# aanna0701/face-recognition-pytorch

Measured on AMD Instinct MI355X. Metric: train imgs/sec IR-50-layout ResNet50 + ArcFace/PartialFC head, 112x112, higher is better.
Workload: dtype bf16

## Files before the change

face-recognition-pytorch_amd/frhip/csrc/igemm_halo.hip:

```cpp
#include "igemm_halo.h"
#include "igemm_halo_wide.h"
#include "frhip.h"

namespace frhip {

#ifndef FRHIP_CLOCK_STAMP
#define FRHIP_CLOCK_STAMP 0
#endif
#if FRHIP_CLOCK_STAMP
__device__ unsigned long long g_clock_stamps[2 * 8192];
#endif

template <typename T, int WM, int WN, int MT, int HBUFS, bool XF = false, bool LEAN = false>
__device__ __forceinline__ void halo_body(const HaloGeom& g, const void* __restrict__ a, const void* __restrict__ b,
                                          void* __restrict__ out, const void* __restrict__ res, float* __restrict__ stats,
                                          const EpiBnRed& br, char* smem, int mtile, int ntile) {
    typedef HaloTile<T, WM, WN, MT, HBUFS> Tile;
    HaloMainloop<T, WM, WN, MT, HBUFS, XF> ml;
#if FRHIP_CLOCK_STAMP
    const unsigned long long t0 = __builtin_amdgcn_s_memtime(), r0 = __builtin_amdgcn_s_memrealtime();
#endif
    ml.run(g, a, b, smem, mtile, ntile);
#if FRHIP_CLOCK_STAMP
    if (threadIdx.x == 0) {
        const unsigned long long t1 = __builtin_amdgcn_s_memtime(), r1 = __builtin_amdgcn_s_memrealtime();
        g_clock_stamps[2 * (blockIdx.x & 8191)] = t1 - t0;
        g_clock_stamps[2 * (blockIdx.x & 8191) + 1] = r1 - r0;
    }
#endif
    if constexpr (FRHIP_ABL & 16) {
        if (g.M >= 0) {
#pragma unroll
            for (int i = 0; i < 4; ++i)
#pragma unroll
                for (int j = 0; j < MT; ++j) asm volatile("" :: "v"(ml.acc[i][j]));
            return;
        }
    }
    const int wave = wave_id();
    const int wm = wave / WN, wn = wave % WN;
    const int m0 = mtile * Tile::BM + wm * Tile::WROWS, n0 = ntile * Tile::BN + wn * 64;
    EpiOperands<T, Tile::WROWS> eo;
    if constexpr (LEAN) {
        eo.fetch_fast(res, stats ? br.y : nullptr, g.M, g.Nout, m0, n0);
        const char* mine = ml.template stage_out<T>(smem);
        nt_epilogue_store_fast<T, WM, WN, Tile::WROWS, Tile::THREADS, Tile::BN>(mine, Tile::template stage_pitch<T>(), smem, g.M, g.Nout,
                                                                                out, res != nullptr, stats, br, eo, mtile, ntile);
    } else {
        eo.fetch(res, (stats || br.gelu_bwd) ? br.y : nullptr, g.M, g.Nout, m0, n0, br.res_h, br.res_w, &br.map);
        const char* mine = ml.template stage_out<T>(smem);
        nt_epilogue_store<T, WM, WN, Tile::WROWS, Tile::THREADS, Tile::BN>(mine, Tile::template stage_pitch<T>(), smem, g.M, g.Nout,
                                                                           out, res != nullptr, stats, br, eo, mtile, ntile, m0, n0);
    }
}

template <typename T, int WM, int WN, int MT, int HBUFS, bool XF = false, bool LEAN = false>
__global__ __launch_bounds__(64 * WM * WN, 2) void halo_kernel(HaloGeom g, const void* __restrict__ a,
                                                                         const void* __restrict__ b, void* __restrict__ out,
                                                                         const void* __restrict__ res, float* __restrict__ stats,
                                                                         EpiBnRed br, int mtiles, int ntiles) {
    extern __shared__ __attribute__((aligned(16))) char smem[];
    const uint32_t lin = xcd_remap(blockIdx.x, gridDim.x);
    const int ntile = (int)(lin % (uint32_t)ntiles), mtile = (int)(lin / (uint32_t)ntiles);
    halo_body<T, WM, WN, MT, HBUFS, XF, LEAN>(g, a, b, out, res, stats, br, smem, mtile, ntile);
}

template <bool LEAN>
__global__ __launch_bounds__(256, 2) void halo_wide_kernel(HaloGeom g, const void* __restrict__ a, const void* __restrict__ b,
                                                           void* __restrict__ out, const void* __restrict__ res,
                                                           float* __restrict__ stats, EpiBnRed br, int mtiles, int ntiles) {
    typedef HaloWideTile Tile;
    typedef bf16_t T;
    extern __shared__ __attribute__((aligned(16))) char smem[];
    const uint32_t lin = xcd_remap(blockIdx.x, gridDim.x);
    const int ntile = (int)(lin % (uint32_t)ntiles), mtile = (int)(lin / (uint32_t)ntiles);
    const int m_tile0 = mtile * Tile::BM;
    HaloWideMainloop ml;
#if FRHIP_CLOCK_STAMP
    const unsigned long long t0 = __builtin_amdgcn_s_memtime(), r0 = __builtin_amdgcn_s_memrealtime();
#endif
    ml.run(g, a, b, smem, m_tile0, ntile);
#if FRHIP_CLOCK_STAMP
    if (threadIdx.x == 0) {
        const unsigned long long t1 = __builtin_amdgcn_s_memtime(), r1 = __builtin_amdgcn_s_memrealtime();
        g_clock_stamps[2 * (blockIdx.x & 8191)] = t1 - t0;
        g_clock_stamps[2 * (blockIdx.x & 8191) + 1] = r1 - r0;
    }
#endif
    const int m0 = m_tile0 + wave_id() * Tile::WROWS;
#pragma unroll
    for (int half = 0; half < 2; ++half) {
        const int n0 = ntile * Tile::BN + half * 64;
        EpiOperands<T, Tile::WROWS> eo;
        if constexpr (LEAN) {
            eo.fetch_fast(res, stats ? br.y : nullptr, g.M, g.Nout, m0, n0);
            const char* mine = ml.stage_out(smem, half);
            nt_epilogue_store_fast<T, 4, 1, Tile::WROWS, Tile::THREADS, 64>(mine, Tile::stage_pitch, smem, g.M, g.Nout, out, res != nullptr,
                                                                            stats, br, eo, mtile, ntile * 2 + half);
        } else {
            eo.fetch(res, (stats || br.gelu_bwd) ? br.y : nullptr, g.M, g.Nout, m0, n0, br.res_h, br.res_w, &br.map);
            const char* mine = ml.stage_out(smem, half);
            nt_epilogue_store<T, 4, 1, Tile::WROWS, Tile::THREADS, 64>(mine, Tile::stage_pitch, smem, g.M, g.Nout, out, res != nullptr,
                                                                       stats, br, eo, mtile, ntile * 2 + half, m0, n0);
        }
    }
}

int g_epi_lean = 1;

bool halo_lean_pick(int family, long long M, int Nout, const EpiBnRed& br) {
    if (family == HALO_WIDE) return g_epi_lean && epi_lean_ok(true, M, Nout, HaloWideTile::BM, HaloWideTile::BN, br);
    typedef HaloTile<bf16_t, 4, 1, 4, 1> Tile;
    return family == HALO_4WAVE && g_epi_lean && epi_lean_ok(true, M, Nout, Tile::BM, Tile::BN, br);
}

static int halo_wide_launch(const HaloGeom& g, const void* a, const void* b, void* out, const void* res, float* stats,
                            const EpiBnRed& br, hipStream_t stream) {
    typedef HaloWideTile Tile;
    const int mtiles = (g.M + Tile::BM - 1) / Tile::BM, ntiles = (g.Nout + Tile::BN - 1) / Tile::BN;
    const bool lean = halo_lean_pick(HALO_WIDE, g.M, g.Nout, br);
    auto kern = lean ? halo_wide_kernel<true> : halo_wide_kernel<false>;
    if (set_dynamic_lds(reinterpret_cast<const void*>(kern), Tile::LDS, "igemm_halo")) return FRHIP_ELAUNCH;
    hipLaunchKernelGGL(kern, dim3(mtiles * ntiles), dim3(Tile::THREADS), Tile::LDS, stream, g, a, b, out, res, stats, br, mtiles, ntiles);
    return check_launch("igemm_halo_wide");
}

template <typename T, int WM, int WN, int MT, int HBUFS, bool XF = false>
static int halo_launch(const HaloGeom& g, const void* a, const void* b, void* out, const void* res, float* stats,
                       const EpiBnRed& br, hipStream_t stream) {
    typedef HaloTile<T, WM, WN, MT, HBUFS> Tile;
    const int mtiles = (g.M + Tile::BM - 1) / Tile::BM, ntiles = (g.Nout + Tile::BN - 1) / Tile::BN;
    const int lds = Tile::template lds_bytes<T>();
    constexpr bool HAS_LEAN = sizeof(T) == 2 && WM == 4 && WN == 1 && MT == 4 && HBUFS == 1;
    bool lean = false;
    if constexpr (HAS_LEAN) lean = halo_lean_pick(HALO_4WAVE, g.M, g.Nout, br);
    auto kern = halo_kernel<T, WM, WN, MT, HBUFS, XF, false>;
    if constexpr (HAS_LEAN) { if (lean) kern = halo_kernel<T, WM, WN, MT, HBUFS, XF, true>; }
    if (set_dynamic_lds(reinterpret_cast<const void*>(kern), lds, "igemm_halo")) return FRHIP_ELAUNCH;
    hipLaunchKernelGGL(kern, dim3(mtiles * ntiles), dim3(Tile::THREADS), lds, stream, g, a, b, out, res, stats, br, mtiles, ntiles);
    return check_launch("igemm_halo");
}

static int g_halo_enabled = 1;

bool halo_applicable(int dtype, int h, int w, int c, int k, int r, int s, int stride, int pad) {
    const int bke = NT_ROWB / (dtype == FRHIP_DT_BF16 ? 2 : 4);
    return g_halo_enabled && r == 3 && s == 3 && stride == 1 && pad == 1 && w <= 56 && (c % bke) == 0 && (k % 8) == 0 &&
           (dtype == FRHIP_DT_BF16 || dtype == FRHIP_DT_F32);
}

static int g_halo_wide_dirs = 2;
static int halo_config(int dtype, int c, int k);
static int halo_config_w(int dtype, int w, int c, int k, int sign) {
    if ((g_halo_wide_dirs & (sign > 0 ? 1 : 2)) && dtype == FRHIP_DT_BF16 && w <= HaloWideTile::MAXW &&
        (k % 128) == 0 && (c % 64) == 0 && c >= 128 && (g_halo_enabled & 3) == 1)
        return 3;
    return halo_config(dtype, c, k);
}
static int halo_config(int dtype, int c, int k) {
    const int es = dtype == FRHIP_DT_BF16 ? 2 : 4;
    const int nchunks = c / (NT_ROWB / es);
    const bool narrow = (k % 128) != 0;
    if (dtype == FRHIP_DT_BF16) {
        const int mode = g_halo_enabled & 3;
        const bool two_per_cu = mode == 2 || (mode != 3 && nchunks <= 8);
        if (two_per_cu || narrow) return (nchunks == 1 || two_per_cu) ? 0 : 1;
        return 2;
    }
    return narrow ? 1 : 2;
}

int halo_family(int dtype, int w, int c, int k, int sign) {
    if (halo_config_w(dtype, w, c, k, sign) == 3) return HALO_WIDE;
    const int cfg = halo_config(dtype, c, k);
    if (dtype == FRHIP_DT_BF16 && cfg == 0) return HALO_4WAVE;
    return cfg == 1 ? HALO_8X1 : HALO_4X2;
}

bool halo_lean_applies(int dtype, int n, int h, int w, int c, int k, int sign) {
    if (!g_epi_lean || dtype != FRHIP_DT_BF16) return false;
    const long long M = 1LL * n * h * w;
    const int cfg = halo_config_w(dtype, w, c, k, sign) == 3 ? 3 : halo_config(dtype, c, k);
    const int bn = cfg == 3 ? HaloWideTile::BN : 64;
    if (cfg != 3 && cfg != 0) return false;
    return M % 256 == 0 && k % bn == 0 && M * k * 2 < 0x7fffffffLL;
}

int halo_stat_rows(int, int m, int, int, int, int) { return (m + 255) / 256; }

bool halo_xf_applicable(int dtype, int h, int w, int c, int k, int r, int s, int stride, int pad) {
    return dtype == FRHIP_DT_BF16 && halo_applicable(dtype, h, w, c, k, r, s, stride, pad) && halo_config(dtype, c, k) == 0;
}

int halo_run(int dtype, const void* a, const void* b, void* out, const void* res, float* stats, const EpiBnRed& br,
             int n, int h, int w, int c, int k, int sign, hipStream_t stream, const float* xf_scale, const float* xf_shift, void* xf_out) {
    const int es = dtype == FRHIP_DT_BF16 ? 2 : 4;
    const long long ab = 1LL * n * h * w * c * es, bb = 1LL * k * 9 * c * es;
    if (ab > 0x7fffffffLL || bb > 0x7fffffffLL) { set_error("igemm_halo: tensor exceeds the 2 GiB buffer window"); return FRHIP_EINVAL; }
    HaloGeom g;
    g.H = h; g.W = w; g.C = c; g.M = n * h * w; g.Nout = k; g.Ktot = 9 * c; g.sign = sign;
    g.a_bytes = (uint32_t)ab; g.b_bytes = (uint32_t)bb;
    g.xf_scale = xf_scale; g.xf_shift = xf_shift; g.xf_out = xf_out;
    g.d_hw = make_fastdiv((uint32_t)(h * w)); g.d_w = make_fastdiv((uint32_t)w);
    const int cfg = halo_config(dtype, c, k);
    if (xf_scale) {
        if (dtype != FRHIP_DT_BF16 || cfg != 0) { set_error("igemm_halo: operand transform not available for this shape"); return FRHIP_EINVAL; }
        return halo_launch<bf16_t, 4, 1, 4, 1, true>(g, a, b, out, res, stats, br, stream);
    }
    const int family = halo_family(dtype, w, c, k, sign);
    if (family == HALO_WIDE) return halo_wide_launch(g, a, b, out, res, stats, br, stream);
    if (family == HALO_4WAVE) return halo_launch<bf16_t, 4, 1, 4, 1>(g, a, b, out, res, stats, br, stream);
    return by_dtype(dtype, "igemm_halo", [&](auto t) {
        typedef decltype(t) T;
        return family == HALO_8X1 ? halo_launch<T, 8, 1, 2, 2>(g, a, b, out, res, stats, br, stream)
                                  : halo_launch<T, 4, 2, 4, 2>(g, a, b, out, res, stats, br, stream);
    });
}

}

#if FRHIP_CLOCK_STAMP
extern "C" int frhip_dbg_clock_read(unsigned long long* host, int pairs) {
    if (pairs > 8192) pairs = 8192;
    return hipMemcpyFromSymbol(host, HIP_SYMBOL(frhip::g_clock_stamps), sizeof(unsigned long long) * 2 * pairs) == hipSuccess ? 0 : -1;
}
#endif

extern "C" int frhip_set_epi_lean(int enabled) {
    const int old = frhip::g_epi_lean;
    if (enabled >= 0) frhip::g_epi_lean = enabled != 0;
    return old;
}

extern "C" int frhip_set_halo_wide_dirs(int dirs) {
    const int old = frhip::g_halo_wide_dirs;
    if (dirs >= 0) frhip::g_halo_wide_dirs = dirs & 3;
    return old;
}

extern "C" int frhip_set_conv_halo(int enabled) {
    const int old = frhip::g_halo_enabled;
    frhip::g_halo_enabled = enabled & 3;
    return old;
}
```

include/frhip.h:

```cpp
#ifndef FRHIP_H
#define FRHIP_H
#include <stddef.h>
#include <stdint.h>

#ifdef __cplusplus
extern "C" {
#endif

#ifndef FRHIP_STREAM_T
#define FRHIP_STREAM_T
#ifdef __HIP_PLATFORM_AMD__
#include <hip/hip_runtime_api.h>
typedef hipStream_t frhip_stream_t;
#else
typedef void* frhip_stream_t;
#endif
#endif

#define FRHIP_OK 0
#define FRHIP_EINVAL (-1)
#define FRHIP_ELAUNCH (-2)
#define FRHIP_DT_BF16 0
#define FRHIP_DT_F32 1

const char* frhip_last_error(void);
int frhip_abi_version(void);
int frhip_spin(long long ticks, frhip_stream_t stream);

int frhip_nt_block_m(int k);
int frhip_conv_stat_rows(int dtype, int m, int k, int h, int w, int c, int r, int s, int stride, int pad);
int frhip_set_wgrad_taps9(int enabled);
int frhip_set_wgrad_mask_table(int enabled);
int frhip_wgrad_mask_table_period(int h, int w);
int frhip_set_conv_halo(int enabled);
int frhip_set_halo_wide_dirs(int dirs);
int frhip_set_epi_lean(int enabled);
int frhip_set_ew_batch(int enabled);
int frhip_set_nt_tile(int tile);
int frhip_conv_fwd_affine(int dtype, const void* x, const void* w, void* y, const float* scale, const float* shift, int relu,
                          const void* residual, int n, int h, int wd, int c, int k, int r, int s, int stride, int pad,
                          frhip_stream_t stream);
int frhip_conv_fwd(int dtype, const void* x, const void* w, void* y, float* stats_partial,
                   int n, int h, int wd, int c, int k, int r, int s, int stride, int pad, frhip_stream_t stream);
int frhip_conv_dgrad(int dtype, const void* dy, const void* wt, void* dx, const void* residual,
                     int n, int h, int wd, int c, int k, int r, int s, int stride, int pad, frhip_stream_t stream);
int frhip_dgrad_stat_rows(int dtype, int n, int h, int wd, int c, int k, int r, int s, int stride, int pad);
int frhip_dgrad_route(int dtype, int n, int h, int wd, int c, int k, int r, int s, int stride, int pad, int residual_stride, int bnred,
                      int out[5]);
int frhip_conv_dgrad_bnred(int dtype, const void* dy, const void* wt, void* dx, const void* residual,
                           const void* y_bn, const float* mean, const float* invstd, const float* mask_scale,
                           const float* mask_shift, float* stats_partial, int n, int h, int wd, int c, int k,
                           int r, int s, int stride, int pad, frhip_stream_t stream);
int frhip_conv_dgrad_fused(int dtype, const void* dy, const void* wt, void* dx, const void* residual, int residual_stride,
                           const void* y_bn, const float* mean, const float* invstd, const float* mask_scale,
                           const float* mask_shift, float* stats_partial, int n, int h, int wd, int c, int k,
                           int r, int s, int stride, int pad, frhip_stream_t stream);
int frhip_conv_dgrad_fused_rs(int dtype, const void* dy, const void* wt, void* dx, const void* residual, int residual_stride,
                              const void* y_bn, const float* mean, const float* invstd, const float* mask_scale,
                              const float* mask_shift, const float* rowscale, int rows_per, float keep_scale,
                              float* stats_partial, int n, int h, int wd, int c, int k, int r, int s, int stride, int pad,
                              frhip_stream_t stream);
int frhip_conv_wgrad(int dtype, const void* dy, const void* x, float* dw, int n, int h, int w, int c,
                     int k, int r, int s, int stride, int pad, int splits, float* workspace, size_t workspace_bytes,
                     frhip_stream_t stream);
int frhip_conv_wgrad_chain_ok(int dtype, int n, int h, int w, int c, int k, int r, int s, int stride, int pad);
int frhip_conv_wgrad_chain(int dtype, const void* dy, const void* x, int n, int h, int w, int c, int k, float* slabs,
                           size_t slab_bytes, float* prev_dw, const float* prev_slabs, int prev_k, int prev_c, int prev_splits,
                           int* splits_out, frhip_stream_t stream);
int frhip_conv_wgrad_chain_finish(float* dw, float* slabs, int k, int c, int splits, frhip_stream_t stream);
int frhip_wgrad_plan(int dtype, int n, int h, int w, int c, int kc, int ldp, int r, int s, int stride, int pad, int splits,
                     int have_workspace, size_t workspace_bytes, int overwrite, int transform, int* plan_out);
int frhip_linear_fwd(int dtype, const void* a, const void* w, const float* bias, void* out, void* act_out,
                     float* stats_partial, int m, int n, int k, frhip_stream_t stream);
int frhip_linear_dgrad_gelu(int dtype, const void* dy, const void* wt, const void* pre, void* dx, float* stats_partial,
                            int m, int n, int k, frhip_stream_t stream);
int frhip_gemm_nt(int dtype, const void* a, const void* b, void* out, int m, int n, int k, int splits,
                  int atomic_f32, frhip_stream_t stream);
int frhip_gemm_nt_splitk(int dtype, const void* a, const void* b, const float* bias, float* out, int m, int n, int k,
                         int splits, float* slabs, size_t slab_bytes, frhip_stream_t stream);
int frhip_gemm_tn(int dtype, const void* p, const void* q, float* out, int m, int kc, int ldp, int c,
                  int splits, float* workspace, size_t workspace_bytes, frhip_stream_t stream);
int frhip_gemm_tn_overwrite(int dtype, const void* p, const void* q, float* out, int m, int kc, int ldp, int c,
                            float* workspace, size_t workspace_bytes, frhip_stream_t stream);

int frhip_colreduce_blocks(int rows, int c, int dtype);
int frhip_colstats(int dtype, const void* x, int rows, int c, float* partial, frhip_stream_t stream);
int frhip_bn_finalize(const float* partial, int nparts, float* scratch, int c, float count,
                      const float* gamma, const float* beta, float* running_mean, float* running_var,
                      float momentum, float eps, float* mean, float* invstd, float* scale, float* shift,
                      frhip_stream_t stream);
int frhip_bn_eval_affine(int c, const float* gamma, const float* beta, const float* running_mean,
                         const float* running_var, float eps, float* scale, float* shift, frhip_stream_t stream);
int frhip_bn_standin_state(int c, const float* gamma, const float* beta, float k, float* mean, float* invstd, float* scale,
                           float* shift, frhip_stream_t stream);
int frhip_bn_apply(int dtype, const void* y, const float* scale, const float* shift, const void* res,
                   const float* res_scale, const float* res_shift, int relu, void* out, int rows, int c,
                   frhip_stream_t stream);
int frhip_bn_bwd_reduce(int dtype, const void* dout, const void* y, const float* mean, const float* invstd,
                        const float* mask_scale, const float* mask_shift, int rows, int c, float* partial,
                        frhip_stream_t stream);
int frhip_bn_bwd_finalize(const float* partial, int nparts, float* scratch, int c, float count,
                          const float* gamma, const float* mean, const float* invstd, float* dgamma,
                          float* dbeta, float* ca, float* cb, float* cc, frhip_stream_t stream);
int frhip_bn_eval_state(int c, const float* gamma, const float* beta, const float* running_mean, const float* running_var, float eps,
                        float* mean, float* invstd, float* scale, float* shift, frhip_stream_t stream);
int frhip_bn_bwd_finalize_eval(const float* partial, int nparts, float* scratch, int c, float count,
                               const float* gamma, const float* mean, const float* invstd, float* dgamma,
                               float* dbeta, float* ca, float* cb, float* cc, frhip_stream_t stream);
int frhip_bn_bwd_apply(int dtype, const void* dout, const void* y, const float* ca, const float* cb,
                       const float* cc, const float* mask_scale, const float* mask_shift, void* dy,
                       int rows, int c, frhip_stream_t stream);
int frhip_bn_apply_rs(int dtype, const void* y, const float* scale, const float* shift, const void* res, const float* rowscale,
                      int rows_per, void* out, int rows, int c, frhip_stream_t stream);
int frhip_bn_bwd_reduce_rs(int dtype, const void* dout, const void* y, const float* mean, const float* invstd, const float* rowscale,
                           int rows_per, int rows, int c, float* partial, frhip_stream_t stream);
int frhip_bn_bwd_apply_rs(int dtype, const void* dout, const void* y, const float* ca, const float* cb, const float* cc,
                          const float* rowscale, int rows_per, void* dy, int rows, int c, frhip_stream_t stream);
int frhip_sum_partials(const float* partial, int nparts, int c, int which, float* out_accum, frhip_stream_t stream);
int frhip_add_bias(float* x, const float* bias, int rows, int c, frhip_stream_t stream);
int frhip_cast_from_f32(int dtype, const float* src, void* dst, size_t n, frhip_stream_t stream);
int frhip_cast_to_f32(int dtype, const void* src, float* dst, size_t n, frhip_stream_t stream);

int frhip_stem_im2col(int dtype, const float* x, void* col, int b, int h, int w, int stride, frhip_stream_t stream);
int frhip_bn_relu_maxpool_fwd(int dtype, const void* y, const float* scale, const float* shift, void* out,
                              uint8_t* argmax, int b, int h, int w, int c, frhip_stream_t stream);
int frhip_maxpool_bwd(int dtype, const void* dpool, const uint8_t* argmax, void* da, int b, int h, int w,
                      int c, frhip_stream_t stream);

int frhip_pack_wt(int dtype, const float* w, void* wt, int k, int rs, int c, frhip_stream_t stream);
int frhip_transpose2d(int dtype_in, int dtype_out, const void* in, void* out, int rows, int cols, int ld_out,
                      frhip_stream_t stream);
int frhip_pack_stem(int dtype, const float* w, void* wp, int k, int kin, int kp, frhip_stream_t stream);
int frhip_unpack_stem_grad(const float* dwp, float* dw, int k, int kin, int kp, frhip_stream_t stream);
int frhip_fc_permute(int dtype, const float* w, void* wp, int nout, int c, int hw, frhip_stream_t stream);
int frhip_fc_unpermute_grad(const float* dwp, float* dw, int nout, int c, int hw, frhip_stream_t stream);
int frhip_pfc_sample_max_local(void);
int frhip_pfc_sample(const int64_t* labels, int n, long long class_start, int num_local, const float* u, int num_sample,
                     int64_t* index_out, int* rel_out, int64_t* n_positive, frhip_stream_t stream);
int frhip_gather_rows(const float* src, const int64_t* index, float* dst, int n, int d, frhip_stream_t stream);
int frhip_scatter_rows(const float* src, const int64_t* index, float* dst, int n, int d, frhip_stream_t stream);

int frhip_head_dw_ok(int dtype, int n, int classes, int d);
int frhip_head_dw(int dtype, const void* dt, int ldt, const void* ehat, const void* what, const float* wnorm, float* dw,
                  int n, int classes, int d, float out_scale, frhip_stream_t stream);
int frhip_l2norm_rows(int dtype, const float* x, void* xhat, float* norms, int rows, int d, float eps,
                      frhip_stream_t stream);
int frhip_l2norm_bwd(int dtype, const float* dxhat, const void* xhat, const float* norms, float* dx,
                     int rows, int d, float out_scale, frhip_stream_t stream);
int frhip_l2norm_bwd_norm(int dtype, const float* dxhat, const void* xhat, const float* norms, const float* dnorm, float* dx,
                          int rows, int d, float out_scale, frhip_stream_t stream);
int frhip_head_groups(int num_classes);
int frhip_head_fwd(int dtype, const void* ehat, const void* what, const int* labels, int n, int classes,
                   int d, float s, float m, float* part_max, float* part_sum, float* ztarget,
                   float* rowmax, float* rowsum, frhip_stream_t stream);
int frhip_head_rescale(float* rowsum, const float* local_max, const float* global_max, int n, frhip_stream_t stream);
int frhip_head_target_prob(const float* ztarget, const int* labels, const float* rowmax, const float* rowsum,
                           float* q, int n, frhip_stream_t stream);
int frhip_head_pack_stats(const float* ztarget, const int* labels, const float* rowmax, const float* rowsum,
                          float* packed, int n, frhip_stream_t stream);
int frhip_head_merge_stats(const float* gathered, int world_size, int n, float* rowmax, float* rowsum, float* q,
                           frhip_stream_t stream);
int frhip_head_loss(const float* q, int n, float* loss, frhip_stream_t stream);
int frhip_head_bwd_dt(int dtype, const void* ehat, const void* what, const int* labels, int n, int classes,
                      int d, float s, float m, const float* rowmax, const float* rowsum, float gscale,
                      const float* upstream, void* dt, int ldt, void* dtt, int ldtt, frhip_stream_t stream);

#define FRHIP_MARGIN_ARCFACE 0
#define FRHIP_MARGIN_COSFACE 1
typedef struct { int kind; int easy; float s, m, filter_thr; } frhip_margin_t;
int frhip_head_fwd_ex(int dtype, const void* ehat, const void* what, const int* labels, int n, int classes,
                      int d, const frhip_margin_t* margin, float* part_max, float* part_sum, float* ztarget,
                      float* rowmax, float* rowsum, frhip_stream_t stream);
int frhip_head_bwd_dt_ex(int dtype, const void* ehat, const void* what, const int* labels, int n, int classes,
                         int d, const frhip_margin_t* margin, const float* rowmax, const float* rowsum, float gscale,
                         const float* upstream, void* dt, int ldt, void* dtt, int ldtt, frhip_stream_t stream);

typedef struct { float s, eps; const float* m_ang; const float* m_add; } frhip_margin_rows_t;
int frhip_adaface_margins(const float* norms, int n, double m, double h, double t_alpha, double eps, int update, float* batch_mean,
                          float* batch_std, float* m_ang, float* m_add, frhip_stream_t stream);
int frhip_magface_margins(const float* norms, int n, double l_a, double u_a, double l_m, double u_m, float* m_ang, float* m_add,
                          float* reg, frhip_stream_t stream);
int frhip_magface_norm_grad(const float* norms, const float* packed, int world_size, int n, const float* rowmax, const float* rowsum,
                            float s, float eps, double l_a, double u_a, double l_m, double u_m, double lambda_g, double gscale,
                            const float* upstream, double out_scale, float* dnorm, frhip_stream_t stream);
int frhip_head_fwd_rows(int dtype, const void* ehat, const void* what, const int* labels, int n, int classes,
                        int d, const frhip_margin_rows_t* margin, float* part_max, float* part_sum, float* ztarget,
                        float* rowmax, float* rowsum, frhip_stream_t stream);
int frhip_head_bwd_dt_rows(int dtype, const void* ehat, const void* what, const int* labels, int n, int classes,
                           int d, const frhip_margin_rows_t* margin, const float* rowmax, const float* rowsum, float gscale,
                           const float* upstream, void* dt, int ldt, void* dtt, int ldtt, frhip_stream_t stream);

int frhip_head_sub_max(void);
int frhip_head_fwd_sub(int dtype, const void* ehat, const void* what, const int* labels, int n, int classes, int d,
                       int subcenters, const frhip_margin_t* margin, float* part_max, float* part_sum, float* ztarget,
                       int* tsub, float* rowmax, float* rowsum, frhip_stream_t stream);
int frhip_head_fwd_sub_rows(int dtype, const void* ehat, const void* what, const int* labels, int n, int classes, int d,
                            int subcenters, const frhip_margin_rows_t* margin, float* part_max, float* part_sum,
                            float* ztarget, int* tsub, float* rowmax, float* rowsum, frhip_stream_t stream);
int frhip_head_bwd_dt_sub(int dtype, const void* ehat, const void* what, const int* labels, int n, int classes, int d,
                          int subcenters, const frhip_margin_t* margin, const float* rowmax, const float* rowsum,
                          float gscale, const float* upstream, void* dt, int ldt, int ldp, void* dtt, int ldtt,
                          frhip_stream_t stream);
int frhip_head_bwd_dt_sub_rows(int dtype, const void* ehat, const void* what, const int* labels, int n, int classes, int d,
                               int subcenters, const frhip_margin_rows_t* margin, const float* rowmax, const float* rowsum,
                               float gscale, const float* upstream, void* dt, int ldt, int ldp, void* dtt, int ldtt,
                               frhip_stream_t stream);

int frhip_conv_bnrelu_fusable(int dtype, int h, int wd, int c, int k, int r, int s, int stride, int pad);
int frhip_conv_fwd_bnrelu(int dtype, const void* x, const float* in_scale, const float* in_shift, const void* w, void* y,
                          float* stats_partial, void* act_out, int n, int h, int wd, int c, int k, int r, int s, int stride,
                          int pad, frhip_stream_t stream);
int frhip_conv_wgrad_bnrelu_fusable(int dtype, int n, int h, int w, int c, int k, int r, int s, int stride, int pad);
int frhip_conv_wgrad_bnrelu(int dtype, const void* dy, const void* x, const float* in_scale, const float* in_shift,
                            float* dw, int n, int h, int w, int c, int k, int r, int s, int stride, int pad, int splits,
                            float* workspace, size_t workspace_bytes, frhip_stream_t stream);

int frhip_quant_fp8_weights(const float* w, void* w8, float* scale, int k, int rowlen, frhip_stream_t stream);
typedef struct { const float* w; void* w8; float* scale; int32_t k, rowlen, row_begin, pad_; } frhip_q8w;
int frhip_quant_fp8_weights_multi(const frhip_q8w* table, int ntensors, int nrows, frhip_stream_t stream);
int frhip_fp8_saturation(int op);
int frhip_quant_fp8(int dtype, const void* x, void* x8, size_t n, float inv_scale, frhip_stream_t stream);
int frhip_bn_apply_q8(int dtype, const void* y, const float* scale, const float* shift, const void* res,
                      const float* res_scale, const float* res_shift, int relu, void* out, void* out8, float inv_q,
                      int rows, int c, frhip_stream_t stream);
int frhip_conv_fwd_fp8(const void* x8, const void* w8, const float* wscale, float act_scale, void* y,
                       float* stats_partial, int n, int h, int wd, int c, int k, int r, int s, int stride, int pad,
                       frhip_stream_t stream);
int frhip_fp8_stat_rows(int m, int k);
int frhip_fp8_conv_stat_rows(int m, int k, int h, int w, int c, int r, int s, int stride, int pad);
int frhip_set_fp8_halo(int enabled);
int frhip_linear_fwd_fp8(const void* a8, const void* w8, const float* wscale, float act_scale, const float* bias,
                         void* out, float* stats_partial, int m, int n, int k, frhip_stream_t stream);

typedef struct frhip_cpb_block {
    const void* coords;
    const void* index;
    const void* w0;
    const void* b0;
    const void* w2;
    const void* logit_scale;
    void* bias;
    void* scale;
    const void* dbias;
    const void* dscale;
    void* dw0;
    void* db0;
    void* dw2;
    void* dlogit_scale;
    int entries, tokens, heads, pad_;
} frhip_cpb_block;
int frhip_cpb_limits(int* max_entries, int* max_heads, int* hidden);
int frhip_cpb_scratch_floats(int nblocks);
int frhip_cpb_fwd(const frhip_cpb_block* blocks_dev, int nblocks, float* scratch, frhip_stream_t stream);
int frhip_cpb_bwd(const frhip_cpb_block* blocks_dev, int nblocks, float* scratch, frhip_stream_t stream);

int frhip_margin_fwd(float* logits, const int64_t* labels, int n, int c, float s, float m, int kind, float* tsave,
                     frhip_stream_t stream);
int frhip_margin_bwd(const float* gout, const int64_t* labels, const float* tsave, int n, int c, float s, float m,
                     int kind, float* gin, frhip_stream_t stream);
int frhip_margin_fwd_ex(float* logits, const int64_t* labels, int n, int c, const frhip_margin_t* margin, float* tsave,
                        uint64_t* filtered, frhip_stream_t stream);
int frhip_margin_bwd_ex(const float* gout, const int64_t* labels, const float* tsave, const uint64_t* filtered, int n, int c,
                        const frhip_margin_t* margin, float* gin, frhip_stream_t stream);
int frhip_margin_fwd_rows(const float* logits, const int64_t* labels, int n, int c, const frhip_margin_rows_t* margin, float* out,
                          frhip_stream_t stream);
int frhip_margin_bwd_rows(const float* gout, const float* logits, const int64_t* labels, int n, int c,
                          const frhip_margin_rows_t* margin, float* gin, frhip_stream_t stream);
int frhip_rows_max(const float* x, int n, int c, float* rowmax, frhip_stream_t stream);
int frhip_rows_exp_sum(float* x, int n, int c, const float* rowmax, float* rowsum, frhip_stream_t stream);
int frhip_rows_normalize(float* x, int n, int c, const float* rowsum, const int64_t* labels, float* ptarget,
                         frhip_stream_t stream);
int frhip_ce_grad(float* p, int n, int c, const int64_t* labels, float inv_n, const float* upstream,
                  frhip_stream_t stream);

int frhip_winattn_fwd(int dtype, const void* qkv, const float* bias, const float* scale, void* out, int b, int h,
                      int w, int c, int heads, int ws, int shift, frhip_stream_t stream);
int frhip_winattn_bwd(int dtype, const void* qkv, const void* dout, const float* bias, const float* scale,
                      void* dqkv, float* dbias, float* dscale, int b, int h, int w, int c, int heads,
                      int ws, int shift, float* workspace, size_t workspace_bytes, frhip_stream_t stream);
int frhip_winattn_bwd_colsum(int dtype, const void* qkv, const void* dout, const float* bias, const float* scale,
                             void* dqkv, float* dbias, float* dscale, float* dqkv_colsum, int b, int h, int w, int c,
                             int heads, int ws, int shift, float* workspace, size_t workspace_bytes, frhip_stream_t stream);
int frhip_winattn_bwd_qvbias(int dtype, const void* qkv, const void* dout, const float* bias, const float* scale,
                             void* dqkv, float* dbias, float* dscale, float* dq_bias, float* dv_bias, int b, int h, int w,
                             int c, int heads, int ws, int shift, float* workspace, size_t workspace_bytes, frhip_stream_t stream);
int frhip_set_winattn_mfma(int enabled);
int frhip_bias_gelu_fwd(int dtype, void* y, const float* bias, void* act_out, int rows, int c, frhip_stream_t stream);
int frhip_gelu_bwd(int dtype, const void* da, const void* h, void* dh, size_t n, frhip_stream_t stream);

int frhip_pair_score(const float* e1, const float* e2, const int64_t* labels, int n, int d, double* scores,
                     int* hist_idx, int* hist_genuine, int* hist_imposter, frhip_stream_t stream);
int frhip_cross_score(const float* e, const int64_t* labels, int n, int d, double* scores, double* pair_labels,
                      int* hist_idx, int* hist_genuine, int* hist_imposter, frhip_stream_t stream);
int frhip_cross_hist(const float* e, const int64_t* labels, int64_t n, int d, int64_t i0, int64_t i1, uint64_t* hist_genuine,
                     uint64_t* hist_imposter, uint64_t* thr_genuine, uint64_t* thr_imposter, frhip_stream_t stream);
int frhip_gallery_topk(const float* probe, const float* gallery, const int64_t* exclude, int64_t p, int64_t g, int d, int k,
                       int64_t g0, int64_t g1, double* top_score, int64_t* top_index, void* workspace, size_t workspace_bytes,
                       frhip_stream_t stream);
int frhip_gallery_topk_workspace(int64_t p, int k, int64_t* bytes);

int frhip_stem_blocks(int b, int h, int w);
int frhip_set_stem_scatter(int enabled);
int frhip_stem_stats(int dtype, const float* x, const void* wp, int b, int h, int w, float* partial, frhip_stream_t stream);
int frhip_stem_fwd(int dtype, const float* x, const void* wp, const float* scale, const float* shift, void* pooled,
                   uint8_t* argmax, int b, int h, int w, frhip_stream_t stream);
int frhip_stem_bwd_reduce(int dtype, const float* x, const void* wp, const void* dpool, const uint8_t* argmax,
                          const float* mean, const float* invstd, const float* scale, const float* shift, int b, int h,
                          int w, float* partial, frhip_stream_t stream);
int frhip_stem_bwd_wgrad(int dtype, const float* x, const void* wp, const void* dpool, const uint8_t* argmax,
                         const float* ca, const float* cb, const float* cc, const float* scale, const float* shift, int b,
                         int h, int w, float* slabs, float* dw, frhip_stream_t stream);
int frhip_stem_gram_floats(void);
int frhip_stem_gram_blocks(int b, int h, int w);
int frhip_stem_gram(int dtype, const float* x, int b, int h, int w, float* partial, float* gram, frhip_stream_t stream);
int frhip_stem_bwd_wgrad_gram(int dtype, const float* x, const void* wp, const void* dpool, const void* pooled,
                              const uint8_t* argmax, const float* gram, const float* ca, const float* cb, const float* cc,
                              int b, int h, int w, float* slabs, float* dw, frhip_stream_t stream);
int frhip_stem_dx(int dtype, const float* x, const void* wp, const void* dpool, const uint8_t* argmax, const void* pooled,
                  const float* ca, const float* cb, const float* cc, int b, int h, int w, float* dx, frhip_stream_t stream);
int frhip_stem_dx_s2(int dtype, const void* dy0, const void* wp, int kp, int b, int h, int w, float* dx, frhip_stream_t stream);

typedef struct { const float* w; void* wc; void* wt; int32_t k, rs, c, tile_begin; } frhip_wprep;
int frhip_prep_conv_weights(int dtype, const frhip_wprep* table, int ntensors, int ntiles, frhip_stream_t stream);

int frhip_dropout_mask(int dtype, void* mask, size_t n, float keep, long long seed, frhip_stream_t stream);

int frhip_augment_u8(const uint8_t* in, float* out, const int32_t* flip, const int32_t* holes, int nholes,
                     int b, int hin, int win, int size, frhip_stream_t stream);
int frhip_augment_u8_lut(const uint8_t* in, const uint8_t* lut, float* out, const int32_t* flip, const int32_t* holes,
                         int nholes, int b, int hin, int win, int size, frhip_stream_t stream);
int frhip_motion_blur_u8(const uint8_t* in, uint8_t* out, const uint8_t* lut, const float* kernels, const int32_t* ksize,
                         int b, int h, int w, frhip_stream_t stream);
int frhip_iso_noise_scratch_doubles(int b);
int frhip_iso_noise_u8(const uint8_t* in, uint8_t* out, double* scratch, const float* params, const int32_t* lum_noise,
                       const float* color_noise, const uint64_t* seeds, int b, int h, int w, frhip_stream_t stream);

#define FRHIP_SGD_CHUNK 65536
#define FRHIP_SGD_MAX_GROUPS 8
typedef struct { float lr, weight_decay, momentum, clip; } frhip_sgd_group;
typedef struct { float* p; const float* g; float* m; uint32_t n; uint32_t group; } frhip_sgd_chunk;
int frhip_sgd_clip_coef(const frhip_sgd_chunk* chunks, int nchunks, const frhip_sgd_group* groups_host, int ngroups,
                        float max_norm, float* partial, float* coef_out, frhip_stream_t stream);
int frhip_sgd_multi(const frhip_sgd_chunk* chunks, int nchunks, const frhip_sgd_group* groups_host, int ngroups,
                    const float* clip_coef, frhip_stream_t stream);

typedef struct { float lr, beta1, beta2, eps, weight_decay, bc1, bc2, clip; } frhip_adamw_group;
typedef struct { float* p; const float* g; float* m; float* v; uint32_t n; uint32_t group; } frhip_adamw_chunk;
int frhip_adamw_clip_coef(const frhip_adamw_chunk* chunks, int nchunks, const frhip_adamw_group* groups_host, int ngroups,
                          float max_norm, float* partial, float* coef_out, frhip_stream_t stream);
int frhip_adamw_multi(const frhip_adamw_chunk* chunks, int nchunks, const frhip_adamw_group* groups_host, int ngroups,
                      const float* clip_coef, frhip_stream_t stream);

#ifdef __cplusplus
}
#endif
#endif
```

Measured before the change: 22980.

## Route fused BN-ReLU halo conv into split or pre-pass launches by grid size

Adds a routing heuristic for the halo conv that applies BN+ReLU to its input while also writing the activated tensor. When there are enough M tiles, it splits the launch. One column of tiles applies the transform and writes the activation, and a second launch covers the remaining columns using that materialised activation, so the transform is not repeated in every column tile. For smaller grids it instead runs a standalone bn_apply pass followed by a plain halo conv. This removes redundant per-column transform work and the writer race, at the cost of an extra launch and a dependency on ordering within the stream.

Measured after the change: 23240 (median of 4 runs). Within noise of the previous version (+1.1%).

```diff
diff --git a/face-recognition-pytorch_amd/frhip/csrc/conv_bnrelu_route.h b/face-recognition-pytorch_amd/frhip/csrc/conv_bnrelu_route.h
--- /dev/null
+++ b/face-recognition-pytorch_amd/frhip/csrc/conv_bnrelu_route.h
@@ -0,0 +1,22 @@
+#pragma once
+
+namespace frhip {
+
+enum BnReluRoute { BNRELU_FUSED = 0, BNRELU_SPLIT = 1, BNRELU_PASS = 2 };
+
+constexpr int BNRELU_BM = 256, BNRELU_BN = 64;
+
+inline int conv_bnrelu_route(long long M, int W, int C, int K, bool act_out, int cus, int forced) {
+    (void)W; (void)C;
+    const long long mtiles = (M + BNRELU_BM - 1) / BNRELU_BM;
+    const int ncols = (K + BNRELU_BN - 1) / BNRELU_BN;
+    if (!act_out) return BNRELU_FUSED;
+    if (forced == BNRELU_FUSED || forced == BNRELU_PASS) return forced;
+    if (ncols < 2) return BNRELU_FUSED;
+    if (forced == BNRELU_SPLIT) return BNRELU_SPLIT;
+    if (ncols < 4) return BNRELU_FUSED;
+    const long long slots = 2LL * (cus > 0 ? cus : 256);
+    return 2 * mtiles >= slots ? BNRELU_SPLIT : BNRELU_PASS;
+}
+
+}
diff --git a/face-recognition-pytorch_amd/frhip/csrc/igemm_halo.hip b/face-recognition-pytorch_amd/frhip/csrc/igemm_halo.hip
--- a/face-recognition-pytorch_amd/frhip/csrc/igemm_halo.hip
+++ b/face-recognition-pytorch_amd/frhip/csrc/igemm_halo.hip
@@ -1,5 +1,6 @@
 #include "igemm_halo.h"
 #include "igemm_halo_wide.h"
+#include "conv_bnrelu_route.h"
 #include "frhip.h"
 
 namespace frhip {
@@ -58,10 +59,10 @@
 __global__ __launch_bounds__(64 * WM * WN, 2) void halo_kernel(HaloGeom g, const void* __restrict__ a,
                                                                          const void* __restrict__ b, void* __restrict__ out,
                                                                          const void* __restrict__ res, float* __restrict__ stats,
-                                                                         EpiBnRed br, int mtiles, int ntiles) {
+                                                                         EpiBnRed br, int col0, int ncols) {
     extern __shared__ __attribute__((aligned(16))) char smem[];
     const uint32_t lin = xcd_remap(blockIdx.x, gridDim.x);
-    const int ntile = (int)(lin % (uint32_t)ntiles), mtile = (int)(lin / (uint32_t)ntiles);
+    const int ntile = col0 + (int)(lin % (uint32_t)ncols), mtile = (int)(lin / (uint32_t)ncols);
     halo_body<T, WM, WN, MT, HBUFS, XF, LEAN>(g, a, b, out, res, stats, br, smem, mtile, ntile);
 }
 
@@ -127,9 +128,11 @@
 
 template <typename T, int WM, int WN, int MT, int HBUFS, bool XF = false>
 static int halo_launch(const HaloGeom& g, const void* a, const void* b, void* out, const void* res, float* stats,
-                       const EpiBnRed& br, hipStream_t stream) {
+                       const EpiBnRed& br, hipStream_t stream, int col0 = 0, int ncols = 0) {
     typedef HaloTile<T, WM, WN, MT, HBUFS> Tile;
     const int mtiles = (g.M + Tile::BM - 1) / Tile::BM, ntiles = (g.Nout + Tile::BN - 1) / Tile::BN;
+    if (ncols == 0) { col0 = 0; ncols = ntiles; }
+    if (col0 < 0 || ncols < 1 || col0 + ncols > ntiles) { set_error("igemm_halo: channel columns outside the output"); return FRHIP_EINVAL; }
     const int lds = Tile::template lds_bytes<T>();
     constexpr bool HAS_LEAN = sizeof(T) == 2 && WM == 4 && WN == 1 && MT == 4 && HBUFS == 1;
     bool lean = false;
@@ -137,11 +140,12 @@
     auto kern = halo_kernel<T, WM, WN, MT, HBUFS, XF, false>;
     if constexpr (HAS_LEAN) { if (lean) kern = halo_kernel<T, WM, WN, MT, HBUFS, XF, true>; }
     if (set_dynamic_lds(reinterpret_cast<const void*>(kern), lds, "igemm_halo")) return FRHIP_ELAUNCH;
-    hipLaunchKernelGGL(kern, dim3(mtiles * ntiles), dim3(Tile::THREADS), lds, stream, g, a, b, out, res, stats, br, mtiles, ntiles);
+    hipLaunchKernelGGL(kern, dim3(mtiles * ncols), dim3(Tile::THREADS), lds, stream, g, a, b, out, res, stats, br, col0, ncols);
     return check_launch("igemm_halo");
 }
 
 static int g_halo_enabled = 1;
+static int g_bnrelu_route = -1;
 
 bool halo_applicable(int dtype, int h, int w, int c, int k, int r, int s, int stride, int pad) {
     const int bke = NT_ROWB / (dtype == FRHIP_DT_BF16 ? 2 : 4);
@@ -205,6 +209,20 @@
     const int cfg = halo_config(dtype, c, k);
     if (xf_scale) {
         if (dtype != FRHIP_DT_BF16 || cfg != 0) { set_error("igemm_halo: operand transform not available for this shape"); return FRHIP_EINVAL; }
+        typedef HaloTile<bf16_t, 4, 1, 4, 1> Tile;
+        static_assert(Tile::BM == BNRELU_BM && Tile::BN == BNRELU_BN, "conv_bnrelu_route.h plans for this tile");
+        const int route = conv_bnrelu_route(g.M, w, c, k, xf_out != nullptr, device_cu_count(), g_bnrelu_route);
+        if (route == BNRELU_PASS) {
+            if (const int rc = frhip_bn_apply(dtype, a, xf_scale, xf_shift, nullptr, nullptr, nullptr, 1, xf_out, g.M, c, stream)) return rc;
+            return halo_run(dtype, xf_out, b, out, res, stats, br, n, h, w, c, k, sign, stream, nullptr, nullptr, nullptr);
+        }
+        if (route == BNRELU_SPLIT) {
+            const int ntiles = (k + Tile::BN - 1) / Tile::BN;
+            if (const int rc = halo_launch<bf16_t, 4, 1, 4, 1, true>(g, a, b, out, res, stats, br, stream, 0, 1)) return rc;
+            HaloGeom g2 = g;
+            g2.xf_scale = g2.xf_shift = nullptr; g2.xf_out = nullptr;
+            return halo_launch<bf16_t, 4, 1, 4, 1>(g2, xf_out, b, out, res, stats, br, stream, 1, ntiles - 1);
+        }
         return halo_launch<bf16_t, 4, 1, 4, 1, true>(g, a, b, out, res, stats, br, stream);
     }
     const int family = halo_family(dtype, w, c, k, sign);
@@ -238,6 +256,16 @@
     return old;
 }
 
+extern "C" int frhip_set_conv_bnrelu_route(int route) {
+    const int old = frhip::g_bnrelu_route;
+    if (route >= -1 && route <= frhip::BNRELU_PASS) frhip::g_bnrelu_route = route;
+    return old;
+}
+
+extern "C" int frhip_conv_bnrelu_route(int n, int h, int wd, int c, int k, int have_act_out, int cus) {
+    return frhip::conv_bnrelu_route(1LL * n * h * wd, wd, c, k, have_act_out != 0, cus, frhip::g_bnrelu_route);
+}
+
 extern "C" int frhip_set_conv_halo(int enabled) {
     const int old = frhip::g_halo_enabled;
     frhip::g_halo_enabled = enabled & 3;
diff --git a/include/frhip.h b/include/frhip.h
--- a/include/frhip.h
+++ b/include/frhip.h
@@ -210,6 +210,8 @@
 int frhip_conv_fwd_bnrelu(int dtype, const void* x, const float* in_scale, const float* in_shift, const void* w, void* y,
                           float* stats_partial, void* act_out, int n, int h, int wd, int c, int k, int r, int s, int stride,
                           int pad, frhip_stream_t stream);
+int frhip_set_conv_bnrelu_route(int route);
+int frhip_conv_bnrelu_route(int n, int h, int wd, int c, int k, int have_act_out, int cus);
 int frhip_conv_wgrad_bnrelu_fusable(int dtype, int n, int h, int w, int c, int k, int r, int s, int stride, int pad);
 int frhip_conv_wgrad_bnrelu(int dtype, const void* dy, const void* x, const float* in_scale, const float* in_shift,
                             float* dw, int n, int h, int w, int c, int k, int r, int s, int stride, int pad, int splits,
```
